# gmlewis/moonbit-flate

Hardware: AMD Instinct MI355X
Metric: GiB/s uncompressed throughput (encode), 64 KiB blocks, deflate-fast (higher is better)
Workload: dtype u8; 1 GPU; 16384 x 65536 B independent streams per GPU (1.000 GiB/GPU), S-text, deflate-fast, parity not checked in this run; streams_per_gpu=16384, stream_len=65536, kind=text, compressed_bytes_per_gpu=488295363, gather=none, parity_checked_streams=0

## Files before the change

### moonbit-flate_amd/build.py

```python
import os
import subprocess
import sys

HERE = os.path.dirname(os.path.abspath(__file__))
ROOT = os.path.dirname(HERE)
CSRC = os.path.join(HERE, "csrc")
LIB_DIR = os.path.join(HERE, "lib")
LIB_PATH = os.path.join(LIB_DIR, "libflate_hip.so")

SOURCES = ["lz77_kernels.hip",  "huff_pack_kernels.hip", "compact_kernels.hip",
           "inflate_kernels.hip", "splice_kernels.hip", "flate_api.hip", "flate_api_deflate.hip", "flate_api_inflate.hip", "gather.hip", "checksum.hip",
           "frame_kernels.hip", "chain_kernels.hip", "bgzf_kernels.hip", "bgzf_range_kernels.hip", "gzip_kernels.hip", "one_kernels.hip", "one_seek_kernels.hip", "gzfile_kernels.hip", "zip_kernels.hip", "flate_api_zip.hip", "synth.cpp"]
HEADERS = ["flate_common.h", "flate_kernels.h", "flate_ctx.h", "api_checks.h", "deflate_plan.h", "inflate_route.h", "checksum_clip.h", "bgzf_rule.h", "bgzf_range_rule.h", "gzip_rule.h", "gzfile_rule.h", "deflate_block_rule.h", "window_compose.h", "seek_index_rule.h", "zip_rule.h", "zip_kernels.h", "block_scan.h", "chain_rule.h", "chain_walk.h", "carve.h", "lz77_device.h",
           "inflate_spec_kernel.inc", "inflate_stream_kernel.inc", "one_probe_kernel.inc", os.path.join(ROOT, "include", "flate_hip.h")]


GROUPS = {
    "lz77": ["lz77_kernels.hip", "lz77_device.h", "flate_api_deflate.hip", "deflate_plan.h"],
    "huff": ["huff_pack_kernels.hip", "compact_kernels.hip", "splice_kernels.hip", "flate_api_deflate.hip", "deflate_plan.h", "block_scan.h"],
    "inflate": ["inflate_kernels.hip", "inflate_spec_kernel.inc", "inflate_stream_kernel.inc", "flate_api_inflate.hip",
                "inflate_route.h", "one_probe_kernel.inc", "one_kernels.hip", "one_seek_kernels.hip", "seek_index_rule.h", "gzfile_kernels.hip", "gzfile_rule.h",
                "deflate_block_rule.h", "window_compose.h", "chain_kernels.hip", "chain_walk.h", "chain_rule.h", "carve.h", "block_scan.h"],
    "checksum": ["checksum.hip", "checksum_clip.h", "block_scan.h", "carve.h"],
    "frame": ["frame_kernels.hip", "bgzf_kernels.hip", "bgzf_range_kernels.hip", "bgzf_rule.h", "bgzf_range_rule.h",
              "gzip_kernels.hip", "gzip_rule.h", "gzfile_kernels.hip", "gzfile_rule.h",
              "zip_kernels.hip", "zip_kernels.h", "zip_rule.h", "flate_api_zip.hip", "checksum.hip", "checksum_clip.h", "flate_api_inflate.hip",
              "inflate_route.h", "flate_api_deflate.hip", "deflate_plan.h", "block_scan.h",
              "chain_kernels.hip", "chain_walk.h", "chain_rule.h", "carve.h"],
}
SHARED = ["flate_common.h", "flate_kernels.h", "flate_ctx.h", "api_checks.h", "flate_api.hip"]


def _hash_files(names):
    import hashlib
    h = hashlib.sha256()
    for n in sorted(names):
        f = n if os.path.isabs(n) else os.path.join(CSRC, n)
        if os.path.exists(f):
            h.update(os.path.basename(f).encode() + b"\0")
            h.update(open(f, "rb").read())
    return h.hexdigest()[:12]


def source_hash(flags_by_source=None):
    import hashlib
    everything = SOURCES + [h for h in HEADERS]
    parts = ["all:" + _hash_files(everything)]
    for g, files in GROUPS.items():
        parts.append(g + ":" + _hash_files(files + SHARED))
    if flags_by_source:
        desc = ";".join("%s=%s" % (k, " ".join(v)) for k, v in sorted(flags_by_source.items()))
        parts.append("flags:" + hashlib.sha256(desc.encode()).hexdigest()[:8])
    return ";".join(parts)


def id_component(build_id, group):
    for part in (build_id or "").split(";"):
        k, _, v = part.partition(":")
        if k == group:
            return v
    return None


def _stale(lib_path=None):
    lib_path = lib_path or LIB_PATH
    if not os.path.exists(lib_path):
        return True
    t = os.path.getmtime(lib_path)
    deps = [os.path.join(CSRC, s) for s in SOURCES] + \
           [h if os.path.isabs(h) else os.path.join(CSRC, h) for h in HEADERS]
    return any(os.path.getmtime(d) > t for d in deps if os.path.exists(d))


OBJ_DIR = os.path.join(ROOT, "build", "obj")
TEST_LIB_PATH = os.path.join(LIB_DIR, "libflate_hip_testbuild.so")
TEST_BUILD_FLAGS = {"gather.hip": ["-DFLATE_HIP_TEST_BUILD"]}


def _compile_objects(hipcc, flags_by_source, verbose):
    import hashlib
    from concurrent.futures import ThreadPoolExecutor
    os.makedirs(OBJ_DIR, exist_ok=True)
    hdr_hash = _hash_files([h for h in HEADERS])
    base = ["-O3", "-std=c++17", "--offload-arch=gfx950", "-fPIC", "-I" + os.path.join(ROOT, "include"), "-I" + CSRC]
    build_id = {"flate_api.hip": ["-DFLATE_HIP_BUILD_ID=\"%s\"" % source_hash(flags_by_source)]}
    jobs = []
    for src in SOURCES:
        path = os.path.join(CSRC, src)
        if not os.path.exists(path):
            continue
        flags = base + build_id.get(src, []) + flags_by_source.get(src, [])
        key = hashlib.sha256((hdr_hash + "\0" + " ".join(flags) + "\0").encode() + open(path, "rb").read()).hexdigest()[:16]
        obj = os.path.join(OBJ_DIR, "%s-%s.o" % (os.path.splitext(src)[0], key))
        jobs.append((path, obj, flags))

    def one(job):
        path, obj, flags = job
        if not os.path.exists(obj):
            tmp = "%s.%d.tmp" % (obj, os.getpid())
            cmd = [hipcc] + flags + ["-c", path, "-o", tmp]
            if verbose:
                print(" ".join(cmd), file=sys.stderr)
            subprocess.check_call(cmd)
            os.replace(tmp, obj)
        return obj

    with ThreadPoolExecutor(max_workers=min(8, os.cpu_count() or 1)) as pool:
        return list(pool.map(one, jobs))


def _link(hipcc, objs, out, verbose):
    tmp = "%s.%d.tmp" % (out, os.getpid())
    cmd = [hipcc, "--offload-arch=gfx950", "-fPIC", "-shared"] + objs + ["-o", tmp, "-lpthread", "-ldl"]
    if verbose:
        print(" ".join(cmd), file=sys.stderr)
    subprocess.check_call(cmd)
    os.replace(tmp, out)


def build(force=False, verbose=False):
    if not force and not _stale():
        return LIB_PATH
    os.makedirs(LIB_DIR, exist_ok=True)
    hipcc = os.environ.get("HIPCC", "/opt/rocm/bin/hipcc")
    _link(hipcc, _compile_objects(hipcc, {}, verbose), LIB_PATH, verbose)
    return LIB_PATH


def build_test(force=False, verbose=False):
    if not force and not _stale(TEST_LIB_PATH):
        return TEST_LIB_PATH
    os.makedirs(LIB_DIR, exist_ok=True)
    hipcc = os.environ.get("HIPCC", "/opt/rocm/bin/hipcc")
    _link(hipcc, _compile_objects(hipcc, TEST_BUILD_FLAGS, verbose), TEST_LIB_PATH, verbose)
    return TEST_LIB_PATH


if __name__ == "__main__":
    print(build(force="--force" in sys.argv, verbose=True))
    if "--test" in sys.argv:
        print(build_test(force="--force" in sys.argv, verbose=True))
```

### moonbit-flate_amd/csrc/lz77_device.h

```cpp
#pragma once

#include "flate_kernels.h"

namespace flate {

constexpr int kDenseKeep = 61;
static_assert(kDenseKeep >= 0 && kDenseKeep <= 61, "an event must start at a lane that leaves it a scan lane (a + 2 <= 63)");
#ifndef FLATE_LZ_SWEEP_EVERY
#define FLATE_LZ_SWEEP_EVERY 20480
#endif
#ifndef FLATE_LZ_SPAN_MAX
#define FLATE_LZ_SPAN_MAX 4096
#endif
#ifndef FLATE_LZ_MARKER_BACK
#define FLATE_LZ_MARKER_BACK 36864
#endif
constexpr uint32_t kSweepEvery = FLATE_LZ_SWEEP_EVERY, kSpanMax = FLATE_LZ_SPAN_MAX, kMarkerBack = FLATE_LZ_MARKER_BACK;
static_assert(kMarkerBack > 32768u && kSweepEvery + kSpanMax + 66u + 258u + kMarkerBack < 65536u && kSpanMax >= 64u,
              "16-bit modular table slots: sweep period + batch span + marker distance must stay below 2^16");

FLATE_D uint32_t ld32(const uint8_t *p) {
  uint32_t v;
  __builtin_memcpy(&v, p, 4);
  return v;
}

FLATE_D uint32_t ld_partial(const uint8_t *p, int rem) {
  uint32_t v = p[0];
  if (rem > 1) v |= (uint32_t)p[1] << 8;
  if (rem > 2) v |= (uint32_t)p[2] << 16;
  return v;
}

FLATE_D uint32_t rdlane(uint32_t v, int lane) {
  return (uint32_t)__builtin_amdgcn_readlane((int)v, lane);
}

struct ChunkGeom {
  const uint8_t *stream;
  uint64_t len;
  uint32_t nchunks;
  uint32_t chunk0;
  uint64_t mbase;
};

FLATE_D ChunkGeom stream_geom(const LzParams &P, uint32_t sid) {
  ChunkGeom g;
  uint64_t a = P.in_off[sid], b = P.in_off[sid + 1];
  g.stream = P.in + a;
  g.len = b - a;
  g.chunk0 = P.chunk_base[sid];
  g.nchunks = P.chunk_base[sid + 1] - g.chunk0;
  g.mbase = (uint64_t)g.chunk0 * kMatchCapPerChunk;
  return g;
}

FLATE_D uint64_t lanes_below(int l) { return l >= 64 ? ~0ull : ((1ull << l) - 1ull); }
FLATE_D uint64_t lanes_upto(int l) { return l >= 63 ? ~0ull : ((1ull << (l + 1)) - 1ull); }
FLATE_D int ffs64(uint64_t m) { return m ? __builtin_ctzll(m) : 64; }

template <int CTRL, int ROW_MASK>
FLATE_D uint32_t dpp_or(uint32_t v) {
  return v | (uint32_t)__builtin_amdgcn_update_dpp(0, (int)v, CTRL, ROW_MASK, 0xf, false);
}
FLATE_D uint32_t wave_or(uint32_t v) {
  v = dpp_or<0x111, 0xf>(v);
  v = dpp_or<0x112, 0xf>(v);
  v = dpp_or<0x114, 0xf>(v);
  v = dpp_or<0x118, 0xf>(v);
  v = dpp_or<0x142, 0xa>(v);
  v = dpp_or<0x143, 0xc>(v);
  return rdlane(v, 63);
}

FLATE_D uint4 ld128(const uint8_t *p) {
  uint4 v;
  __builtin_memcpy(&v, p, 16);
  return v;
}

FLATE_D int prefix16(uint4 a, uint4 b) {
  const uint64_t lo = (uint64_t)(a.x ^ b.x) | ((uint64_t)(a.y ^ b.y) << 32);
  const uint64_t hi = (uint64_t)(a.z ^ b.z) | ((uint64_t)(a.w ^ b.w) << 32);
  if (lo) return __builtin_ctzll(lo) >> 3;
  if (hi) return 8 + (__builtin_ctzll(hi) >> 3);
  return 16;
}

constexpr uint32_t kDictEnd = (uint32_t)kMaxStoreBlockSize;
template <bool DICT>
struct HistDict {};
template <>
struct HistDict<true> {
  const uint8_t *dict;
};
template <bool DICT>
struct Hist : HistDict<DICT> {
  const uint8_t *stream;
  FLATE_D uint8_t byte(uint32_t p) const {
    if constexpr (DICT)
      if (p < kDictEnd) return this->dict[p];
    return stream[p];
  }
  FLATE_D uint32_t w32(uint32_t p) const {
    if constexpr (!DICT) return ld32(stream + p);
    if (p >= kDictEnd) return ld32(stream + p);
    if constexpr (DICT)
      if (p + 4u <= kDictEnd) return ld32(this->dict + p);
    return (uint32_t)byte(p) | ((uint32_t)byte(p + 1) << 8) | ((uint32_t)byte(p + 2) << 16) | ((uint32_t)byte(p + 3) << 24);
  }
  FLATE_D uint32_t partial(uint32_t p, int rem) const {
    if constexpr (!DICT) return ld_partial(stream + p, rem);
    if (p >= kDictEnd) return ld_partial(stream + p, rem);
    uint32_t v = byte(p);
    if (rem > 1) v |= (uint32_t)byte(p + 1) << 8;
    if (rem > 2) v |= (uint32_t)byte(p + 2) << 16;
    return v;
  }
  FLATE_D uint4 w128(uint32_t p) const {
    if constexpr (!DICT) return ld128(stream + p);
    if (p >= kDictEnd) return ld128(stream + p);
    if constexpr (DICT)
      if (p + 16u <= kDictEnd) return ld128(this->dict + p);
    return make_uint4(w32(p), w32(p + 4), w32(p + 8), w32(p + 12));
  }
};

template <bool DICT = false>
FLATE_D int extend_match(const uint8_t *src, const Hist<DICT> hist, uint32_t W, int n, int pf,
                         uint32_t cand, int have, uint32_t compat_go, int lane) {
  if (!compat_go && cand + 4 < W) return 4;
  int limit = n - pf;
  if (limit > 258) limit = 258;
  const int o = have + 4 * lane;
  uint32_t x = 0;
  if (o < limit) {
    const int r = limit - o;
    const uint8_t *pa = src + pf + o;
    if constexpr (!DICT) {
      const uint8_t *pb = hist.stream + cand + o;
      x = r >= 4 ? (ld32(pa) ^ ld32(pb)) : (ld_partial(pa, r) ^ ld_partial(pb, r));
    } else {
      const uint32_t pb = cand + (uint32_t)o;
      x = r >= 4 ? (ld32(pa) ^ hist.w32(pb)) : (ld_partial(pa, r) ^ hist.partial(pb, r));
    }
  }
  const uint64_t mm = __ballot(x != 0);
  if (!mm) return limit;
  const int k = __builtin_ctzll(mm);
  return have + 4 * k + (__builtin_ctz(rdlane(x, k)) >> 3);
}

}
```

### moonbit-flate_amd/csrc/lz77_kernels.hip

```cpp
#include <type_traits>

#include "lz77_device.h"

namespace flate {

__global__ __launch_bounds__(64) void lz77_serial_kernel(LzParams P) {
  __shared__ uint32_t table[kTableSize];
  const int lane = threadIdx.x;
  const uint32_t sid = P.stream_ids ? P.stream_ids[blockIdx.x] : blockIdx.x;
  for (int i = lane; i < kTableSize; i += 64) table[i] = 0;
  __syncthreads();
  if (lane != 0) return;

  const ChunkGeom g = stream_geom(P, sid);
  for (uint32_t c = 0; c < g.nchunks; ++c) {
    const uint32_t W = c * (uint32_t)kMaxStoreBlockSize;
    const uint64_t rem = g.len - W;
    const int n = rem < (uint64_t)kMaxStoreBlockSize ? (int)rem : kMaxStoreBlockSize;
    const uint8_t *src = g.stream + W;
    uint2 *mout = P.matches + g.mbase + (uint64_t)c * kMatchCapPerChunk;
    uint32_t nm = 0, sumlen = 0;

    const int s_limit = n - kInputMargin;
    int s = 0;
    uint32_t cv = ld32(src);
    bool done = false;
    while (!done) {
      int skip = 32;
      int next_s = s;
      uint32_t cand = 0;
      for (;;) {
        s = next_s;
        int step = skip >> 5;
        next_s = s + step;
        skip += step;
        if (next_s > s_limit) {
          done = true;
          break;
        }
        uint32_t h = hash4(cv);
        cand = table[h];
        uint32_t now = ld32(src + next_s);
        table[h] = W + (uint32_t)s + 1;
        bool ok = cand != 0 && (W + (uint32_t)s + 1 - cand) <= (uint32_t)kMaxMatchOffset &&
                  ld32(g.stream + (cand - 1)) == cv;
        if (!ok) {
          cv = now;
          continue;
        }
        break;
      }
      if (done) break;
      for (;;) {
        const int pf = s;
        s += 4;
        const uint32_t Ac = cand - 1;
        int limit = n - s;
        if (limit > kMaxMatchTail) limit = kMaxMatchTail;
        int l = 0;
        if (P.compat_go || Ac + 4 >= W) {
          const uint8_t *a = src + s, *b = g.stream + Ac + 4;
          while (l < limit && a[l] == b[l]) ++l;
        }
        mout[nm] = make_uint2((uint32_t)pf, kMatchType | ((uint32_t)(l + 1) << kLengthShift) |
                                                ((W + (uint32_t)pf) - Ac - 1));
        ++nm;
        sumlen += (uint32_t)l + 4;
        s += l;
        if (s >= s_limit) {
          done = true;
          break;
        }
        uint32_t x0 = ld32(src + s - 1), x1 = ld32(src + s);
        table[hash4(x0)] = W + (uint32_t)s;
        uint32_t h1 = hash4(x1);
        cand = table[h1];
        table[h1] = W + (uint32_t)s + 1;
        bool ok = cand != 0 && (W + (uint32_t)s + 1 - cand) <= (uint32_t)kMaxMatchOffset &&
                  ld32(g.stream + (cand - 1)) == x1;
        if (!ok) {
          cv = ld32(src + s + 1);
          s += 1;
          break;
        }
      }
    }
    P.chunk_nmatch[g.chunk0 + c] = nm;
    P.chunk_ntok[g.chunk0 + c] = (uint32_t)n - sumlen + nm;
  }
}


#ifdef FLATE_LZ_STAMPS
#define STAMP(var) const uint64_t var = __builtin_amdgcn_s_memtime()
#define STAMP_ADD(acc, t1, t0) acc += (t1) - (t0)
#else
#define STAMP(var)
#define STAMP_ADD(acc, t1, t0)
#endif


FLATE_D uint64_t same_slot_lanes(uint32_t h, uint64_t among) {
  uint32_t lo = (uint32_t)among, hi = (uint32_t)(among >> 32);
#pragma unroll
  for (int k = 0; k < kTableBits; ++k) {
    uint32_t bm = (uint32_t)((int32_t)(h << (31 - k)) >> 31);
    asm volatile("" : "+v"(bm));
    const uint64_t m = __ballot(bm != 0);
    lo &= ~((uint32_t)m ^ bm);
    hi &= ~((uint32_t)(m >> 32) ^ bm);
  }
  return ((uint64_t)hi << 32) | lo;
}

#ifndef FLATE_LZ_TAG_SLOTS
#define FLATE_LZ_TAG_SLOTS 16384
#endif
constexpr uint32_t kTagSlots = FLATE_LZ_TAG_SLOTS;
static_assert(kTagSlots % 1024 == 0 && kTagSlots <= (uint32_t)kTableSize, "whole rounds of 64 lanes x 16 slots");
FLATE_D uint32_t tag_of(uint32_t cv) { return ((cv * 0x1e35a7bdu) >> 16) & 3u; }
FLATE_D bool tag_says_no(const uint32_t *tags, uint32_t h, uint32_t cv) {
  if (kTagSlots < (uint32_t)kTableSize && h >= kTagSlots) return false;
  return ((tags[h >> 4] >> (2u * (h & 15u))) & 3u) != tag_of(cv);
}
FLATE_D void tag_set(uint32_t *tags, uint32_t h, uint32_t t) {
  if (kTagSlots < (uint32_t)kTableSize && h >= kTagSlots) return;
  const uint32_t sh = 2u * (h & 15u);
  atomicAnd(&tags[h >> 4], ~(3u << sh));
  atomicOr(&tags[h >> 4], t << sh);
}

constexpr int kLzDictStream = 1, kLzDictPrime = 2;
template <bool MULTI, bool GUEST = false, int DMODE = 0, bool HOOKS = false>
FLATE_D void lz77_stream(const LzParams &P, const uint32_t sid, uint16_t *table, const int lane,
                         const uint32_t c_begin = 0, const uint32_t c_end = 0xffffffffu,
                         uint32_t *sweep_io = nullptr, uint32_t *tags = nullptr,
                         const LzDictParams *DP = nullptr) {
  using E = uint16_t;
  constexpr bool PRIME = DMODE == kLzDictPrime, DICT = DMODE == kLzDictStream;
  static_assert(DMODE == 0 || MULTI, "a dictionary puts the payload behind position 65535: modular slots");
  uint32_t prime_w = 0, prime_n = 0;
  if constexpr (PRIME) {
    prime_n = (uint32_t)__builtin_amdgcn_readfirstlane((int)DP->dict_len[sid]);
    prime_w = kDictEnd - prime_n;
  }
  if (tags && c_begin == 0)
    for (int i = lane; i < (int)kTagSlots / 16; i += 64) tags[i] = 0;
  if (c_begin == 0) {
    uint4 *t4 = reinterpret_cast<uint4 *>(table);
    const uint32_t fill = MULTI ? (((prime_w - kMarkerBack + 1u) & 0xffffu) * 0x10001u) : 0u;
    const uint4 z = make_uint4(fill, fill, fill, fill);
    for (int i = lane; i < (int)(kTableSize * sizeof(E) / 16); i += 64) t4[i] = z;
  }
  __syncthreads();
  volatile E *vtable = table;
  constexpr uint32_t kEMask = 0xffffu;
  uint32_t next_sweep = (sweep_io && c_begin != 0) ? *sweep_io : prime_w + kSweepEvery;
  auto sweep = [&](uint32_t R) {
    uint32_t *t32 = reinterpret_cast<uint32_t *>(table);
    const uint32_t marker = (R - kMarkerBack + 1u) & 0xffffu;
    static_assert(kTableSize / 2 % (64 * 16) == 0, "table = whole rounds of 16 dwords per lane");
    for (int i0 = lane; i0 < kTableSize / 2; i0 += 64 * 16) {
      uint32_t w[16];
#pragma unroll
      for (int k = 0; k < 16; ++k) w[k] = t32[i0 + 64 * k];
#pragma unroll
      for (int k = 0; k < 16; ++k) {
        const uint32_t v = w[k];
        const uint32_t d0 = (R + 1u - v) & 0xffffu, d1 = (R + 1u - (v >> 16)) & 0xffffu;
        const uint32_t lo = (d0 == 0 || d0 > 32768u) ? marker : (v & 0xffffu);
        const uint32_t hi = (d1 == 0 || d1 > 32768u) ? marker : (v >> 16);
        t32[i0 + 64 * k] = lo | (hi << 16);
      }
    }
    __syncthreads();
    next_sweep = R + kSweepEvery;
  };

  ChunkGeom g;
  Hist<DICT> hist;
  if constexpr (PRIME) {
    g.stream = DP->dict_buf + DP->dict_at[sid] - prime_w;
    g.len = kDictEnd;
    g.nchunks = 1;
    g.chunk0 = 0;
    g.mbase = 0;
  } else {
    g = stream_geom(P, sid);
  }
  if constexpr (DICT) {
    const uint32_t slot = DP->slot_of[sid];
    hist.dict = DP->dict_buf + DP->dict_at[slot] - (kDictEnd - DP->dict_len[slot]);
    g.stream -= kDictEnd;
    g.len += kDictEnd;
  }
  hist.stream = g.stream;
  const uint16_t *scan_tab = P.scan_off;
  uint32_t pf_sink = 0;
#ifdef FLATE_LZ_FINISH
  const uint64_t fin_t0 = __builtin_amdgcn_s_memrealtime();
#endif

  const uint32_t w0 = (uint32_t)__builtin_amdgcn_readfirstlane((int)P.win0);
  const uint32_t c_stop = c_end < w0 + g.nchunks ? c_end : w0 + g.nchunks;
  for (uint32_t c = c_begin; c < c_stop; ++c) {
    const uint32_t W = PRIME ? prime_w : c * (uint32_t)kMaxStoreBlockSize;
    const uint64_t rem_len = g.len - W;
    const int n = rem_len < (uint64_t)kMaxStoreBlockSize ? (int)rem_len : kMaxStoreBlockSize;
    const uint8_t *src = g.stream + W;
    uint2 *mout = P.matches + g.mbase + (uint64_t)(c - w0) * kMatchCapPerChunk;
    uint32_t nm = 0;
    uint32_t acc_len = 0;
    const int s_limit = n - kInputMargin;

    int s = -1;
    bool sparse = false;
    int scan_base = 0, e_idx = 0;
    bool done = false;
    uint4 own_pre = make_uint4(0, 0, 0, 0);
    bool pre_valid = false;
    int pf_blk = -2;
#ifdef FLATE_LZ_STAMPS
    uint64_t st_load = 0, st_dup = 0, st_ev = 0, st_commit = 0, st_sparse = 0, st_nb = 0, st_ext = 0;
#endif

    const uint64_t spec_full =
        (2ull << lane) | (lane + 2 < 64 ? ((0x00000000ffffffffull << (lane + 2)) | (0x5555555500000000ull << (lane + 2)))
                                        : 0ull);
    auto no_progress = [&]() {
      if (lane == 0) atomicExch(P.status, kStatusNoProgress);
      done = true;
    };
    uint32_t h_nb = 0, h_acc = 0;
    int h_e = 0;
    bool moved = true;
    while (!done) {
      if (!moved) {
        no_progress();
        break;
      }
      if constexpr (HOOKS) h_acc = acc_len, h_e = e_idx;
      if (!sparse) {
        auto dense_batch = [&](auto interior_tag) {
          constexpr bool INTERIOR = decltype(interior_tag)::value;
        STAMP(t0);
        const int B = s - 1;
        if (MULTI) {
          const uint32_t first = W + (uint32_t)(B < 0 ? 0 : B);
          if (first >= next_sweep) sweep(first);
        }
        const int q = B + lane;
        const bool e1 = INTERIOR || (q >= 0 && q + 1 <= s_limit);
        const bool e2 = INTERIOR || (q >= 0 && q + 2 <= s_limit);
        const uint64_t E1 = INTERIOR ? ~0ull : __ballot(e1), E2 = INTERIOR ? ~0ull : __ballot(e2);
        const uint32_t A1 = W + (uint32_t)q + 1;
        uint4 own = make_uint4(0, 0, 0, 0);
        uint32_t h = 0, old = 0;
        bool maybe = false;
        if (e1) {
          own = pre_valid ? own_pre : ld128(src + q);
          h = hash4(own.x);
          maybe = !tags || !tag_says_no(tags, h, own.x);
          if (maybe) old = table[h];
        }
        pre_valid = false;
        const uint32_t dist = MULTI ? ((A1 - old) & 0xffffu) : (A1 - old);
        const bool inr = maybe && (MULTI ? dist != 0 : old != 0) && dist <= (uint32_t)kMaxMatchOffset;
        const uint32_t cand_abs = A1 - 1u - dist;
        uint4 cb = own;
        if (inr) cb = hist.w128(cand_abs);
        if ((B >> 8) != pf_blk) {
          pf_blk = B >> 8;
          int pq = (B & ~255) + 1024 + 4 * lane;
          if (pq > n - 4) pq = n - 4;
          pf_sink = ld32(src + pq);
        }
        uint64_t DUPall = 0, DUP = 0;
        uint64_t eq = 0;
        if (GUEST) {
          eq = same_slot_lanes(h, E1);
          if (!e1) eq = 0;
          DUPall = __ballot((eq & ~(1ull << lane)) != 0);
          DUP = __ballot((eq & lanes_below(lane)) != 0);
        }
        asm volatile("" ::: "memory");
        if (!GUEST && e1) table[h] = (E)A1;
        asm volatile("" ::: "memory");
        const uint32_t rb = (!GUEST && e1) ? (uint32_t)table[h] : (A1 & kEMask);
        asm volatile("" ::: "memory");
        const bool loser = rb != (A1 & kEMask);
        const uint64_t LM = GUEST ? 0ull : __ballot(loser);
        if (!GUEST) DUPall = LM;
        if (LM) {
          const int wl = (int)((rb - (W + (uint32_t)B + 1u)) & kEMask);
          uint64_t m = LM;
          while (m) {
            const int x = __builtin_ctzll(m);
            const int w = (int)rdlane((uint32_t)wl, x);
            const uint64_t Lw = __ballot(loser && wl == w);
            DUPall |= 1ull << w;
            if (__popcll(Lw) == 1)
              DUP |= 1ull << (w > x ? w : x);
            else
              DUP |= Lw | (1ull << w);
            m &= ~Lw;
          }
        }
        STAMP(t1);
        const int bsh = lane + 2;
        uint64_t specR;
        if (E1 == ~0ull && E2 == ~0ull) {
          specR = spec_full;
        } else {
          specR = (E1 & (2ull << lane)) | (bsh < 64 ? (((0x00000000ffffffffull << bsh) & E1) |
                                                       ((0x5555555500000000ull << bsh) & E2))
                                                    : 0ull);
        }
        const uint64_t dupR = DUP & specR;
        const int fd = dupR ? __builtin_ctzll(dupR) : 64;
        const int mlen = inr ? prefix16(own, cb) : 0;
        const uint64_t OK = __ballot(mlen >= 4);
        const bool cross = MULTI && !P.compat_go && cand_abs + 4 < W;
        const int tot_self = cross ? 4 : mlen;
        uint32_t rec_tok = kMatchType | ((uint32_t)(tot_self - 3) << kLengthShift) | (dist - 1u);
        uint32_t ev;
        {
          const uint64_t okR = OK & specR & ~DUP;
          const int fv = okR ? __builtin_ctzll(okR) : 64;
          const int tf = __shfl(tot_self, fv & 63);
          const bool slow = !(fv < fd) || tf >= 16;
          const bool ends = B + fv + tf >= s_limit;
          const int nxt = fv + tf - 1;
#ifdef FLATE_LZ_TERM_SHORTCUT
          const bool off_batch = INTERIOR && fv == 64 && fd == 64;
#else
          constexpr bool off_batch = false;
#endif
          ev = (uint32_t)(fv & 127) | ((uint32_t)tf << 8) | (slow ? 1u << 16 : 0u) |
               (ends ? 1u << 17 : 0u) | ((ends || nxt > kDenseKeep) ? 1u << 18 : 0u) | (off_batch ? 1u << 19 : 0u) |
               ((uint32_t)(nxt & 255) << 24);
        }
        STAMP(t2);

        auto fast_inserts = [&](uint64_t vis) -> uint64_t {
          const uint64_t below_me = vis & lanes_upto(lane);
          const int j = below_me ? 63 - __builtin_clzll(below_me) : 0;
          const int fvj = (int)(__shfl(ev, j) & 127u);
          const int d = lane - j, o = d - 2;
          const bool sched = (d <= 1 || o < 32) ? e1 : (((o & 1) == 0) ? e2 : false);
          return __ballot(below_me != 0 && sched && lane <= fvj);
        };
        uint64_t INS = 0, M = 0, MF = 0;
        uint64_t VISall = 0;
        int a = 0;
        for (;;) {
          uint32_t x, tmp;
          uint64_t VIS = 0, MFl = 0;
          int a_s = __builtin_amdgcn_readfirstlane(a);
          STAMP(tc0);
          asm volatile(
              "1:\n\t"
              "s_nop 1\n\t"
              "v_readlane_b32 %[x], %[ev], %[a]\n\t"
              "s_nop 3\n\t"
              "s_bitcmp1_b32 %[x], 16\n\t"
              "s_cbranch_scc1 2f\n\t"
              "s_bitset1_b64 %[vis], %[a]\n\t"
              "s_and_b32 %[t], %[x], 0x7f\n\t"
              "s_bitset1_b64 %[mf], %[t]\n\t"
              "s_lshr_b32 %[a], %[x], 24\n\t"
              "s_bitcmp1_b32 %[x], 18\n\t"
              "s_cbranch_scc1 2f\n\t"
              "s_nop 1\n\t"
              "v_readlane_b32 %[x], %[ev], %[a]\n\t"
              "s_nop 3\n\t"
              "s_bitcmp1_b32 %[x], 16\n\t"
              "s_cbranch_scc1 2f\n\t"
              "s_bitset1_b64 %[vis], %[a]\n\t"
              "s_and_b32 %[t], %[x], 0x7f\n\t"
              "s_bitset1_b64 %[mf], %[t]\n\t"
              "s_lshr_b32 %[a], %[x], 24\n\t"
              "s_bitcmp1_b32 %[x], 18\n\t"
              "s_cbranch_scc0 1b\n\t"
              "2:\n\t"
              : [x] "=&s"(x), [a] "+s"(a_s), [vis] "+s"(VIS), [mf] "+s"(MFl), [t] "=&s"(tmp)
              : [ev] "v"(ev)
              : "scc");
          a = a_s;
          MF |= MFl;
          STAMP(tc1);
          STAMP_ADD(st_sparse, tc1, tc0);
          VISall |= VIS;
          s = B + a + 1;
          if (!(x & (1u << 16))) {
            if (x & (1u << 17)) done = true;
            break;
          }
#ifdef FLATE_LZ_TERM_SHORTCUT
          if (INTERIOR && (x & (1u << 19)) && a != 0) break;
#endif
          STAMP(tg0);
          const uint64_t FINS = fast_inserts(VISall);
          const uint64_t a_ins = E1 & (1ull << a);
          const int b = a + 2;
          const uint64_t full = 0x55555555ffffffffull << b;
          const uint64_t scanR = ((0x00000000ffffffffull << b) & E1) | ((0x5555555500000000ull << b) & E2);
          const uint64_t R = (E1 & (2ull << a)) | scanR;
          const bool scan_ended = scanR != full;

          uint64_t T = 0, rem = R;
          int f = 64, have = 0;
          uint32_t cand = 0;
          for (;;) {
            const int fv = ffs64(OK & rem & ~DUP), fd = ffs64(DUP & rem);
            if (fv < fd) {
              f = fv;
              cand = rdlane(cand_abs, fv);
              have = (int)rdlane((uint32_t)mlen, fv);
              T |= rem & lanes_upto(fv);
              break;
            }
            if (fd == 64) {
              T |= rem;
              break;
            }
            T |= rem & lanes_below(fd);
            const uint32_t hfd = rdlane(h, fd);
            const uint64_t G = __ballot(e1 && h == hfd) & (INS | FINS | T | a_ins) & lanes_below(fd);
            bool v;
            uint32_t cnd;
            int ml;
            if (G) {
              const int i = 63 - __builtin_clzll(G);
              v = rdlane(own.x, i) == rdlane(own.x, fd);
              cnd = W + (uint32_t)(B + i);
              const uint4 oi = make_uint4(rdlane(own.x, i), rdlane(own.y, i), rdlane(own.z, i),
                                          rdlane(own.w, i));
              const uint4 of = make_uint4(rdlane(own.x, fd), rdlane(own.y, fd), rdlane(own.z, fd),
                                          rdlane(own.w, fd));
              ml = prefix16(of, oi);
            } else {
              v = (OK >> fd) & 1;
              cnd = rdlane(cand_abs, fd);
              ml = (int)rdlane((uint32_t)mlen, fd);
            }
            T |= 1ull << fd;
            if (v) {
              f = fd;
              cand = cnd;
              have = ml;
              break;
            }
            rem &= ~lanes_upto(fd);
          }

          if (f == 64) {
            if (scan_ended) {
              INS |= T | a_ins;
              done = true;
            } else if (a == 0) {
              INS |= T | a_ins;
              sparse = true;
              scan_base = s + 1;
              e_idx = 47;
            }
            break;
          }
          INS |= T | a_ins;
          const int pf = B + f;
          int total;
          if (have < 16)
            total = (!P.compat_go && cand + 4 < W) ? 4 : have;
          else
            total = extend_match(src, hist, W, n, pf, cand, 16, P.compat_go, lane);
          M |= 1ull << f;
          if (lane == f) {
            rec_tok = kMatchType | ((uint32_t)(total - 3) << kLengthShift) | ((W + (uint32_t)pf) - cand - 1);
            acc_len += (uint32_t)total;
          }
          s = pf + total;
          STAMP(tg1);
          STAMP_ADD(st_ext, tg1, tg0);
          if (s >= s_limit) {
            done = true;
            break;
          }
          a = s - 1 - B;
          if (a > kDenseKeep) break;
        }
        M |= MF;
        INS |= fast_inserts(VISall);
        if constexpr (HOOKS) {
          if (P.inject_stall != 0 && ++h_nb == P.inject_stall) {
            s = B + 1, e_idx = h_e, sparse = false, done = false;
            acc_len = h_acc;
            M = MF = INS = 0;
          }
        }
        STAMP(t3);
        if (!done && !sparse) {
          const int qn = s - 1 + lane;
          if (qn + 1 <= s_limit) own_pre = ld128(src + qn);
          pre_valid = true;
        }
        if ((MF >> lane) & 1) acc_len += (uint32_t)tot_self;
        if (!PRIME && ((M >> lane) & 1))
          {
            const unsigned long long rec = (unsigned long long)(uint32_t)q | ((unsigned long long)rec_tok << 32);
            __builtin_nontemporal_store(
                rec, reinterpret_cast<unsigned long long *>(mout + nm + (uint32_t)__popcll(M & lanes_below(lane))));
          }
        nm += (uint32_t)__popcll(M);
        asm volatile("" ::: "memory");
        if (GUEST) {
          if (e1 && ((INS >> lane) & 1) && (eq & INS & ~lanes_upto(lane)) == 0) {
            table[h] = (E)A1;
            if (tags) tag_set(tags, h, tag_of(own.x));
          }
        } else {
          if (e1 && (((DUPall | ~INS) >> lane) & 1)) table[h] = (E)old;
          uint64_t dm = DUPall & INS;
          while (dm) {
            const int k = __builtin_ctzll(dm);
            asm volatile("" ::: "memory");
            if (lane == k) table[h] = (E)A1;
            dm &= dm - 1;
          }
        }
        asm volatile("" ::: "memory");
        STAMP(t4);
        STAMP_ADD(st_dup, t1, t0);
        STAMP_ADD(st_load, t2, t1);
        STAMP_ADD(st_ev, t3, t2);
        STAMP_ADD(st_commit, t4, t3);
#ifdef FLATE_LZ_STAMPS
        st_nb += 1;
#endif
        };
        const int s0 = s;
        if (s - 1 >= 0 && s - 1 + 65 <= s_limit)
          dense_batch(std::true_type{});
        else
          dense_batch(std::false_type{});
        moved = (s != s0) | sparse | done;
      } else {
        const int e = e_idx + lane;
        int p, step;
        if (e < kScanClosedForm) {
          p = scan_base + scan_off_small(e, &step);
        } else {
          const int ec = e < P.scan_len - 1 ? e : P.scan_len - 2;
          const int o0 = scan_tab[ec], o1 = scan_tab[ec + 1];
          p = scan_base + o0 + (e - ec) * 65536;
          step = o1 - o0;
        }
        const bool exists_all = p + step <= s_limit;
        const int p0 = (int)rdlane((uint32_t)p, 0);
        const bool exists = exists_all && (!MULTI || (uint32_t)(p - p0) < kSpanMax);
        const int nall = __popcll(__ballot(exists_all));
        const int nexist = __popcll(__ballot(exists));
        if (nall == 0) break;
        if (MULTI && W + (uint32_t)p0 >= next_sweep) sweep(W + (uint32_t)p0);

        uint32_t cv = 0, h = 0, old = 0;
        if (exists) {
          cv = ld32(src + p);
          h = hash4(cv);
          old = vtable[h];
        }
        const uint32_t A1 = W + (uint32_t)p + 1;
        const uint32_t dist = MULTI ? ((A1 - old) & 0xffffu) : (A1 - old);
        const uint32_t cand_abs = A1 - 1u - dist;
        bool ok = false;
        if (exists && (MULTI ? dist != 0 : old != 0) && dist <= (uint32_t)kMaxMatchOffset)
          ok = hist.w32(cand_abs) == cv;
        const uint64_t V = __ballot(ok);
        const int f0 = ffs64(V);

        const int lim = f0 < nexist - 1 ? f0 : nexist - 1;
        const bool ins = lane <= lim;
        uint64_t C;
        if (GUEST) {
          const uint64_t eqs = same_slot_lanes(h, __ballot(ins));
          C = __ballot(ins && (eqs & ~(1ull << lane)) != 0);
          if (C == 0 && ins) {
            vtable[h] = (E)A1;
            if (tags) tag_set(tags, h, tag_of(cv));
          }
        } else {
          if (ins) vtable[h] = (E)A1;
          const uint32_t rb = ins ? (uint32_t)vtable[h] : (A1 & kEMask);
          C = __ballot(rb != (A1 & kEMask));
        }

        int f = f0;
        uint32_t cand = 0;
        if (C == 0) {
          if (f0 < 64) cand = rdlane(cand_abs, f0);
        } else {
          if (!GUEST && ins) vtable[h] = (E)old;
          f = 64;
          for (int e2 = 0; e2 < nexist; ++e2) {
            const uint32_t he = rdlane(h, e2);
            const uint32_t pe1 = rdlane(A1, e2);
            const uint32_t cur =
                (uint32_t)__builtin_amdgcn_readfirstlane((int)(uint32_t)vtable[he]);
            vtable[he] = (E)pe1;
            if (tags && lane == e2) tag_set(tags, h, tag_of(cv));
            bool v;
            uint32_t cnd;
            if (cur == rdlane(old, e2)) {
              v = (V >> e2) & 1;
              cnd = rdlane(cand_abs, e2);
            } else {
              const uint64_t m = __ballot(exists && (A1 & kEMask) == cur);
              v = false;
              cnd = 0;
              if (m) {
                const int i = __builtin_ctzll(m);
                v = rdlane(cv, i) == rdlane(cv, e2);
                cnd = rdlane(A1, i) - 1u;
              }
            }
            if (v) {
              f = e2;
              cand = cnd;
              break;
            }
          }
        }
        if (f == 64) {
          if (nexist == nall && nall < 64) break;
          if (nexist == 0) {
            no_progress();
            break;
          }
          e_idx += nexist;
          continue;
        }
        const int pf = (int)rdlane((uint32_t)p, f);
        const int total = extend_match(src, hist, W, n, pf, cand, 4, P.compat_go, lane);
        if (!PRIME && lane == 0)
          mout[nm] = make_uint2((uint32_t)pf, kMatchType | ((uint32_t)(total - 3) << kLengthShift) |
                                                  ((W + (uint32_t)pf) - cand - 1));
        ++nm;
        if (lane == 0) acc_len += (uint32_t)total;
        s = pf + total;
        sparse = false;
        if (s >= s_limit) done = true;
      }
    }
    uint32_t sumlen = acc_len;
    for (int d = 32; d >= 1; d >>= 1) sumlen += __shfl_xor(sumlen, d);
    if (pf_sink == 0x9e3779b9u && P.debug) P.debug[0] = pf_sink;
    if (!PRIME && lane == 0) {
      P.chunk_nmatch[g.chunk0 + c - w0] = nm;
      P.chunk_ntok[g.chunk0 + c - w0] = (uint32_t)n - sumlen + nm;
#ifdef FLATE_LZ_STAMPS
      if (P.debug) {
        uint64_t *d = P.debug + (uint64_t)(g.chunk0 + c - w0) * 8;
        d[0] = st_dup; d[1] = st_load; d[2] = st_ev; d[3] = st_commit; d[4] = st_nb; d[5] = nm;
        d[6] = st_ext; d[7] = st_sparse;
      }
#endif
    }
  }
  if (sweep_io) *sweep_io = next_sweep;
#ifdef FLATE_LZ_FINISH
  if (lane == 0 && P.debug && c_begin == 0) {
    uint64_t *d = P.debug + (uint64_t)g.chunk0 * 8;
    d[0] = fin_t0;
    d[1] = __builtin_amdgcn_s_memrealtime();
    d[2] = ((uint64_t)(GUEST ? 1u : 0u) << 32) | blockIdx.x;
  }
#endif
}

FLATE_D void all_lanes_here(const LzParams &P, int lane) {
  const uint64_t here = __ballot(true);
  if (here != ~0ull && lane == (int)__builtin_ctzll(here)) atomicExch(P.status, kStatusLanesLost);
}

struct UqUnit {
  uint32_t q;
  uint32_t c;
  bool ok;
};

template <bool HOOKS>
FLATE_D UqUnit uq_pop(const LzParams &P, const uint32_t push_word, int lane) {
  uint32_t t = 0;
  if (lane == 0) {
    if (push_word != 0 && !(push_word & 0x80000000u)) {
      const uint32_t k = __hip_atomic_fetch_add(P.uq_ctr + 1, 1u, __ATOMIC_RELAXED, __HIP_MEMORY_SCOPE_AGENT);
      bool dropped = false;
      if constexpr (HOOKS) dropped = k + 1u - P.queue_end == P.inject_drop_push;
      if (!dropped)
        __hip_atomic_store(P.uq_ready + k, push_word, __ATOMIC_RELAXED, __HIP_MEMORY_SCOPE_AGENT);
    }
    t = __hip_atomic_fetch_add(P.uq_ctr, 1u, __ATOMIC_RELAXED, __HIP_MEMORY_SCOPE_AGENT);
  }
  t = (uint32_t)__builtin_amdgcn_readfirstlane((int)t);
  const uint32_t units = P.uq_units;
  uint32_t v = 0;
  if (t < units) {
    for (uint32_t polls = 0;; ++polls) {
      uint32_t x = 0;
      if (lane == 0) x = __hip_atomic_load(P.uq_ready + t, __ATOMIC_RELAXED, __HIP_MEMORY_SCOPE_AGENT);
      v = (uint32_t)__builtin_amdgcn_readfirstlane((int)x);
      if (v != 0) break;
      if (polls >= P.spin_limit) break;
      __builtin_amdgcn_s_sleep(16);
    }
    if (v == 0 && lane == 0) atomicExch(P.status, kStatusUqTimeout);
    if (lane == 0) (void)__hip_atomic_load(P.uq_ready + t, __ATOMIC_ACQUIRE, __HIP_MEMORY_SCOPE_AGENT);
    asm volatile("s_waitcnt vmcnt(0)" ::: "memory");
  }
  __syncthreads();
  UqUnit u;
  v = (uint32_t)__builtin_amdgcn_readfirstlane((int)v);
  u.ok = v != 0;
  u.q = (v >> 15) - 1u;
  u.c = v & 0x7fffu;
  return u;
}

__global__ void uq_init_kernel(uint32_t *ready, uint32_t *ctr, uint32_t n_streams, uint32_t n_units) {
  const uint32_t i = blockIdx.x * blockDim.x + threadIdx.x;
  if (i < n_units) ready[i] = i < n_streams ? ((i + 1u) << 15) : 0u;
  if (i == 0) {
    ctr[0] = 0;
    ctr[1] = n_streams;
  }
}

template <bool GUEST, bool HOOKS>
FLATE_D uint32_t uq_run(const LzParams &P, const UqUnit u, uint16_t *table, int lane, uint32_t *tags = nullptr) {
  const uint32_t sid = (uint32_t)__builtin_amdgcn_readfirstlane((int)P.stream_ids[u.q]);
  const uint32_t nch = (uint32_t)__builtin_amdgcn_readfirstlane((int)(P.chunk_base[sid + 1] - P.chunk_base[sid]));
  uint32_t *home = reinterpret_cast<uint32_t *>(P.uq_tables + (size_t)u.q * kTableSize);
  uint32_t *work = reinterpret_cast<uint32_t *>(table);
  uint32_t clock = 0;
  if (u.c != 0) {
    clock = (uint32_t)__builtin_amdgcn_readfirstlane(
        (int)__hip_atomic_load(P.uq_sweep + u.q, __ATOMIC_RELAXED, __HIP_MEMORY_SCOPE_AGENT));
    const uint8_t *stream = P.in + P.in_off[sid];
    const uint32_t W = u.c * (uint32_t)kMaxStoreBlockSize;
    if (tags) {
      for (int i = lane; i < (int)kTagSlots / 16; i += 64) tags[i] = 0;
      __syncthreads();
    }
    static_assert(kTableSize / 2 % (64 * 16) == 0, "table = whole rounds of 16 dwords per lane");
    for (int i0 = lane; i0 < kTableSize / 2; i0 += 64 * 16) {
      uint32_t w[16];
#pragma unroll
      for (int k = 0; k < 16; ++k) w[k] = __hip_atomic_load(home + i0 + 64 * k, __ATOMIC_RELAXED, __HIP_MEMORY_SCOPE_AGENT);
#pragma unroll
      for (int k = 0; k < 16; ++k) work[i0 + 64 * k] = w[k];
      if (tags) {
#pragma unroll
        for (int half = 0; half < 2; ++half) {
          uint32_t cv[16];
#pragma unroll
          for (int j = 0; j < 16; ++j) {
            const uint32_t slot = (w[half * 8 + j / 2] >> (16 * (j & 1))) & 0xffffu;
            const uint32_t back = (W + 1u - slot) & 0xffffu;
            cv[j] = (back != 0u && back <= W) ? ld32(stream + (W - back)) : 0xffffffffu;
          }
#pragma unroll
          for (int j = 0; j < 16; ++j) {
            const uint32_t slot = (w[half * 8 + j / 2] >> (16 * (j & 1))) & 0xffffu;
            const uint32_t back = (W + 1u - slot) & 0xffffu;
            const uint32_t h = 2u * (uint32_t)(i0 + 64 * (half * 8 + j / 2)) + (uint32_t)(j & 1);
            if (back != 0u && back <= W && h < kTagSlots) atomicOr(&tags[h >> 4], tag_of(cv[j]) << (2u * (h & 15u)));
          }
        }
      }
    }
  }
  asm volatile("s_waitcnt vmcnt(0) lgkmcnt(0)" ::: "memory");
  __syncthreads();
  lz77_stream<true, GUEST, 0, HOOKS>(P, sid, table, lane, u.c, u.c + 1, &clock, tags);
  asm volatile("s_waitcnt vmcnt(0) lgkmcnt(0)" ::: "memory");
  __syncthreads();
  if (u.c + 1 < nch) {
    for (int i0 = lane; i0 < kTableSize / 2; i0 += 64 * 16) {
      uint32_t w[16];
#pragma unroll
      for (int k = 0; k < 16; ++k) w[k] = work[i0 + 64 * k];
#pragma unroll
      for (int k = 0; k < 16; ++k) __hip_atomic_store(home + i0 + 64 * k, w[k], __ATOMIC_RELAXED, __HIP_MEMORY_SCOPE_AGENT);
    }
    if (lane == 0) __hip_atomic_store(P.uq_sweep + u.q, clock, __ATOMIC_RELAXED, __HIP_MEMORY_SCOPE_AGENT);
    asm volatile("s_waitcnt vmcnt(0) lgkmcnt(0)" ::: "memory");
    __syncthreads();
    return ((u.q + 1u) << 15) | (u.c + 1u);
  }
  return 0x80000000u | u.q;
}

FLATE_D void table_copy(uint16_t *dst, const uint16_t *src, int lane) {
  const uint32_t *s = reinterpret_cast<const uint32_t *>(src);
  uint32_t *d = reinterpret_cast<uint32_t *>(dst);
  static_assert(kTableSize / 2 % (64 * 16) == 0, "table = whole rounds of 16 dwords per lane");
  for (int i0 = lane; i0 < kTableSize / 2; i0 += 64 * 16) {
    uint32_t w[16];
#pragma unroll
    for (int k = 0; k < 16; ++k) w[k] = s[i0 + 64 * k];
#pragma unroll
    for (int k = 0; k < 16; ++k) d[i0 + 64 * k] = w[k];
  }
}

FLATE_D void dict_snapshot_load(const LzDictParams &DP, uint32_t sid, uint16_t *table, uint32_t *clock, int lane) {
  const uint32_t slot = (uint32_t)__builtin_amdgcn_readfirstlane((int)DP.slot_of[sid]);
  table_copy(table, DP.tables + (size_t)slot * kTableSize, lane);
  *clock = (uint32_t)__builtin_amdgcn_readfirstlane((int)DP.clocks[slot]);
  asm volatile("s_waitcnt vmcnt(0) lgkmcnt(0)" ::: "memory");
  __syncthreads();
}


template <bool MULTI, bool GUEST, bool DICT, bool COUNT, bool HOOKS>
FLATE_D void stream_loop(const LzParams P, uint16_t *table, uint32_t *tags, const LzDictParams *DP, int lane) {
  uint32_t mine = 0;
  for (bool first = true;; first = false) {
    uint32_t q;
    if (GUEST || P.queue) {
      q = 0;
      if (lane == 0) q = atomicAdd(P.queue, 1u);
      q = (uint32_t)__builtin_amdgcn_readfirstlane((int)q);
      if (q >= P.queue_end) break;
    } else {
      if (!first) break;
      q = blockIdx.x;
    }
    __syncthreads();
    if constexpr (DICT) {
      const uint32_t sid = (uint32_t)__builtin_amdgcn_readfirstlane((int)P.stream_ids[q]);
      uint32_t clock = 0;
      dict_snapshot_load(*DP, sid, table, &clock, lane);
      lz77_stream<true, GUEST, kLzDictStream, HOOKS>(P, sid, table, lane, 1, 0xffffffffu, &clock, nullptr, DP);
    } else {
      lz77_stream<MULTI, GUEST, 0, HOOKS>(P, (GUEST || P.stream_ids) ? P.stream_ids[q] : q, table, lane, 0, 0xffffffffu,
                                          nullptr, tags);
    }
    __syncthreads();
    all_lanes_here(P, lane);
    if (COUNT) ++mine;
  }
  if (COUNT && P.taken && lane == 0) __hip_atomic_fetch_add(P.taken, mine, __ATOMIC_RELAXED, __HIP_MEMORY_SCOPE_AGENT);
}

template <bool GUEST, bool COUNT, bool HOOKS>
FLATE_D void unit_loop(const LzParams P, uint16_t *table, uint32_t *tags, int lane) {
  uint32_t push_word = 0;
  uint32_t mine = 0;
  for (;;) {
    const UqUnit u = uq_pop<HOOKS>(P, push_word, lane);
    if (__builtin_amdgcn_readfirstlane((int)u.ok) == 0) break;
    push_word = (uint32_t)__builtin_amdgcn_readfirstlane((int)uq_run<GUEST, HOOKS>(P, u, table, lane, tags));
    all_lanes_here(P, lane);
    if (COUNT) ++mine;
  }
  if (COUNT && P.taken && lane == 0) __hip_atomic_fetch_add(P.taken, mine, __ATOMIC_RELAXED, __HIP_MEMORY_SCOPE_AGENT);
}

template <bool MULTI, bool HOOKS>
__global__ __launch_bounds__(64) void lz77_wave_kernel(LzParams P) {
  __shared__ uint16_t table[kTableSize];
  if (MULTI && P.uq_ready)
    unit_loop<false, true, HOOKS>(P, table, nullptr, threadIdx.x);
  else
    stream_loop<MULTI, false, false, true, HOOKS>(P, table, nullptr, nullptr, threadIdx.x);
}

FLATE_D uint16_t *guest_table(const LzParams &P) {
  return reinterpret_cast<uint16_t *>(P.gtables) + (size_t)blockIdx.x * kTableSize;
}

template <bool MULTI, bool HOOKS>
__global__ __launch_bounds__(64) void lz77_guest_kernel(LzParams P) {
  if (blockIdx.x >= P.gtable_blocks) return;
  __shared__ uint32_t tags[kTagSlots / 16];
  uint16_t *table = guest_table(P);
  const int lane = threadIdx.x;
  if (MULTI && P.uq_ready) {
    unit_loop<true, false, HOOKS>(P, table, tags, lane);
    return;
  }
  stream_loop<MULTI, true, false, false, HOOKS>(P, table, tags, nullptr, lane);
}

template <bool HOOKS>
__global__ __launch_bounds__(64) void lz77_wave_dict_kernel(LzParams P, LzDictParams DP) {
  __shared__ uint16_t table[kTableSize];
  stream_loop<true, false, true, false, HOOKS>(P, table, nullptr, &DP, threadIdx.x);
}

template <bool HOOKS>
__global__ __launch_bounds__(64) void lz77_guest_dict_kernel(LzParams P, LzDictParams DP) {
  if (blockIdx.x >= P.gtable_blocks) return;
  stream_loop<true, true, true, false, HOOKS>(P, guest_table(P), nullptr, &DP, threadIdx.x);
}

__global__ __launch_bounds__(64) void lz77_dict_prime_kernel(LzParams P, LzDictParams DP) {
  __shared__ uint16_t table[kTableSize];
  const int lane = threadIdx.x;
  const uint32_t slot = blockIdx.x;
  uint32_t clock = 0;
  lz77_stream<true, false, kLzDictPrime>(P, slot, table, lane, 0, 1, &clock, nullptr, &DP);
  __syncthreads();
  table_copy(DP.tables + (size_t)slot * kTableSize, table, lane);
  if (lane == 0) DP.clocks[slot] = clock;
}


__global__ __launch_bounds__(64) void lz77_resume_kernel(LzParams P, uint16_t *table_io, uint32_t *clock_io,
                                                          uint32_t nwin, uint32_t rebase, uint32_t forget) {
  __shared__ uint16_t table[kTableSize];
  const int lane = threadIdx.x;
  uint32_t clock = 0;
  if (P.win0 != 0 && forget) {
    const uint32_t W = P.win0 * (uint32_t)kMaxStoreBlockSize;
    const uint32_t fill = ((W - kMarkerBack + 1u) & 0xffffu) * 0x10001u;
    uint4 *dst = reinterpret_cast<uint4 *>(table);
    for (int i = lane; i < (int)(kTableSize * sizeof(uint16_t) / 16); i += 64) dst[i] = make_uint4(fill, fill, fill, fill);
    clock = W + kSweepEvery;
  } else if (P.win0 != 0) {
    table_copy(table, table_io, lane);
    clock = *clock_io - rebase;
    if (rebase) {
      __syncthreads();
      uint32_t *t32 = reinterpret_cast<uint32_t *>(table);
      const uint32_t d16 = rebase & 0xffffu;
      for (int i = lane; i < kTableSize / 2; i += 64) {
        const uint32_t v = t32[i];
        t32[i] = ((v - d16) & 0xffffu) | ((((v >> 16) - d16) & 0xffffu) << 16);
      }
    }
  }
  __syncthreads();
  lz77_stream<true>(P, 0, table, lane, P.win0, P.win0 + nwin, &clock);
  __syncthreads();
  table_copy(table_io, table, lane);
  if (lane == 0) *clock_io = clock;
}

template __global__ void lz77_wave_kernel<false, false>(LzParams);
template __global__ void lz77_wave_kernel<true, false>(LzParams);
template __global__ void lz77_guest_kernel<false, false>(LzParams);
template __global__ void lz77_guest_kernel<true, false>(LzParams);
template __global__ void lz77_wave_dict_kernel<false>(LzParams, LzDictParams);
template __global__ void lz77_guest_dict_kernel<false>(LzParams, LzDictParams);
template __global__ void lz77_wave_kernel<false, true>(LzParams);
template __global__ void lz77_wave_kernel<true, true>(LzParams);
template __global__ void lz77_guest_kernel<false, true>(LzParams);
template __global__ void lz77_guest_kernel<true, true>(LzParams);
template __global__ void lz77_wave_dict_kernel<true>(LzParams, LzDictParams);
template __global__ void lz77_guest_dict_kernel<true>(LzParams, LzDictParams);

}
```

Before: 58.10 GiB/s.

## Precompute two-hop event pairs so the scalar LZ77 chase jumps two events per readlane

Each lane now builds a second packed word that combines its own match event with the event it points to, fetched with one cross-lane shuffle. The serial scalar chase loop reads this pair word, so each dependent v_readlane plus its nop padding advances two events instead of one. This shortens the latency-bound pointer chain through the wavefront. In exchange it adds a shuffle and some bit packing per batch, and the asm hard-codes the new bit layout. A host-side reference model of the chase is added, and the unused FLATE_LZ_TERM_SHORTCUT path is removed.

```diff
diff --git a/moonbit-flate_amd/build.py b/moonbit-flate_amd/build.py
--- a/moonbit-flate_amd/build.py
+++ b/moonbit-flate_amd/build.py
@@ -11,12 +11,12 @@
 SOURCES = ["lz77_kernels.hip",  "huff_pack_kernels.hip", "compact_kernels.hip",
            "inflate_kernels.hip", "splice_kernels.hip", "flate_api.hip", "flate_api_deflate.hip", "flate_api_inflate.hip", "gather.hip", "checksum.hip",
            "frame_kernels.hip", "chain_kernels.hip", "bgzf_kernels.hip", "bgzf_range_kernels.hip", "gzip_kernels.hip", "one_kernels.hip", "one_seek_kernels.hip", "gzfile_kernels.hip", "zip_kernels.hip", "flate_api_zip.hip", "synth.cpp"]
-HEADERS = ["flate_common.h", "flate_kernels.h", "flate_ctx.h", "api_checks.h", "deflate_plan.h", "inflate_route.h", "checksum_clip.h", "bgzf_rule.h", "bgzf_range_rule.h", "gzip_rule.h", "gzfile_rule.h", "deflate_block_rule.h", "window_compose.h", "seek_index_rule.h", "zip_rule.h", "zip_kernels.h", "block_scan.h", "chain_rule.h", "chain_walk.h", "carve.h", "lz77_device.h",
+HEADERS = ["flate_common.h", "flate_kernels.h", "flate_ctx.h", "api_checks.h", "deflate_plan.h", "inflate_route.h", "checksum_clip.h", "bgzf_rule.h", "bgzf_range_rule.h", "gzip_rule.h", "gzfile_rule.h", "deflate_block_rule.h", "window_compose.h", "seek_index_rule.h", "zip_rule.h", "zip_kernels.h", "block_scan.h", "chain_rule.h", "chain_walk.h", "carve.h", "lz77_device.h", "lz77_chase_rule.h",
            "inflate_spec_kernel.inc", "inflate_stream_kernel.inc", "one_probe_kernel.inc", os.path.join(ROOT, "include", "flate_hip.h")]
 
 
 GROUPS = {
-    "lz77": ["lz77_kernels.hip", "lz77_device.h", "flate_api_deflate.hip", "deflate_plan.h"],
+    "lz77": ["lz77_kernels.hip", "lz77_device.h", "lz77_chase_rule.h", "flate_api_deflate.hip", "deflate_plan.h"],
     "huff": ["huff_pack_kernels.hip", "compact_kernels.hip", "splice_kernels.hip", "flate_api_deflate.hip", "deflate_plan.h", "block_scan.h"],
     "inflate": ["inflate_kernels.hip", "inflate_spec_kernel.inc", "inflate_stream_kernel.inc", "flate_api_inflate.hip",
                 "inflate_route.h", "one_probe_kernel.inc", "one_kernels.hip", "one_seek_kernels.hip", "seek_index_rule.h", "gzfile_kernels.hip", "gzfile_rule.h",
diff --git a/moonbit-flate_amd/csrc/lz77_chase_rule.h b/moonbit-flate_amd/csrc/lz77_chase_rule.h
--- /dev/null
+++ b/moonbit-flate_amd/csrc/lz77_chase_rule.h
@@ -0,0 +1,84 @@
+#pragma once
+
+#include <stdint.h>
+
+#if defined(__HIPCC__)
+#define CHASE_HD __host__ __device__ inline
+#else
+#define CHASE_HD inline
+#endif
+
+namespace flate {
+
+constexpr int kDenseKeep = 61;
+static_assert(kDenseKeep >= 0 && kDenseKeep <= 61, "an event must start at a lane that leaves it a scan lane (a + 2 <= 63)");
+
+constexpr uint32_t kEvSlow = 1u << 16, kEvEnds = 1u << 17, kEvStop = 1u << 18;
+constexpr int kEvNextShift = 24;
+
+constexpr uint32_t kPairNone = 1u << 15;
+constexpr int kPairFv1Shift = 8, kPairA1Shift = 19, kPairNextShift = 25;
+static_assert(kDenseKeep < 64 && 63 + 15 - 1 < 128, "a1 takes six bits and the next start lane seven");
+
+CHASE_HD uint32_t chase_pair(uint32_t lane, uint32_t ev_mine, uint32_t ev_next) {
+  const bool stop = (ev_mine & kEvStop) != 0, next_slow = (ev_next & kEvSlow) != 0;
+  const bool two = !stop && !next_slow;
+  const uint32_t last = two ? ev_next : ev_mine;
+#ifndef CHASE_MUTANT_IGNORE_STOP2
+  uint32_t bits = last & (kEvEnds | kEvStop);
+#else
+  uint32_t bits = last & (two ? kEvEnds : (kEvEnds | kEvStop));
+#endif
+  if (!stop && next_slow) bits = kEvSlow | kEvStop;
+  const uint32_t w = (last & 63u) | ((ev_mine & 63u) << kPairFv1Shift) | bits |
+                     ((two ? ev_mine >> kEvNextShift : lane) << kPairA1Shift) |
+                     ((last >> kEvNextShift) << kPairNextShift);
+  return (ev_mine & kEvSlow) ? (kPairNone | kEvSlow) : w;
+}
+
+struct ChaseEnd {
+  uint64_t vis, mf;
+  uint32_t a, exit;
+};
+CHASE_HD uint32_t chase_exit_bits(uint32_t x) { return (x & kEvSlow) ? kEvSlow : (x & kEvEnds); }
+
+CHASE_HD ChaseEnd chase_single(const uint32_t *ev, uint32_t a) {
+  ChaseEnd r = {0, 0, a, 0};
+  for (;;) {
+    const uint32_t x = ev[r.a];
+    r.exit = chase_exit_bits(x);
+    if (x & kEvSlow) return r;
+    r.vis |= 1ull << r.a;
+    r.mf |= 1ull << (x & 63u);
+    r.a = x >> kEvNextShift;
+    if (x & kEvStop) return r;
+  }
+}
+
+CHASE_HD ChaseEnd chase_paired(const uint32_t *ev, const uint32_t *ev2, uint32_t a) {
+  ChaseEnd r = {0, 0, a, 0};
+  for (;;) {
+    const uint32_t x = ev2[r.a];
+    if (x & kPairNone) {
+      const uint32_t y = ev[r.a];
+      r.exit = chase_exit_bits(y);
+      if (y & kEvSlow) return r;
+      r.vis |= 1ull << r.a;
+      r.mf |= 1ull << (y & 63u);
+      r.a = y >> kEvNextShift;
+      if (y & kEvStop) return r;
+      continue;
+    }
+    r.exit = chase_exit_bits(x);
+#ifndef CHASE_MUTANT_DROP_MIDDLE
+    r.vis |= (1ull << r.a) | (1ull << ((x >> kPairA1Shift) & 63u));
+#else
+    r.vis |= 1ull << r.a;
+#endif
+    r.mf |= (1ull << ((x >> kPairFv1Shift) & 63u)) | (1ull << (x & 63u));
+    r.a = x >> kPairNextShift;
+    if (x & kEvStop) return r;
+  }
+}
+
+}
diff --git a/moonbit-flate_amd/csrc/lz77_device.h b/moonbit-flate_amd/csrc/lz77_device.h
--- a/moonbit-flate_amd/csrc/lz77_device.h
+++ b/moonbit-flate_amd/csrc/lz77_device.h
@@ -1,11 +1,10 @@
 #pragma once
 
 #include "flate_kernels.h"
+#include "lz77_chase_rule.h"
 
 namespace flate {
 
-constexpr int kDenseKeep = 61;
-static_assert(kDenseKeep >= 0 && kDenseKeep <= 61, "an event must start at a lane that leaves it a scan lane (a + 2 <= 63)");
 #ifndef FLATE_LZ_SWEEP_EVERY
 #define FLATE_LZ_SWEEP_EVERY 20480
 #endif
diff --git a/moonbit-flate_amd/csrc/lz77_kernels.hip b/moonbit-flate_amd/csrc/lz77_kernels.hip
--- a/moonbit-flate_amd/csrc/lz77_kernels.hip
+++ b/moonbit-flate_amd/csrc/lz77_kernels.hip
@@ -331,15 +331,11 @@
           const bool slow = !(fv < fd) || tf >= 16;
           const bool ends = B + fv + tf >= s_limit;
           const int nxt = fv + tf - 1;
-#ifdef FLATE_LZ_TERM_SHORTCUT
-          const bool off_batch = INTERIOR && fv == 64 && fd == 64;
-#else
-          constexpr bool off_batch = false;
-#endif
           ev = (uint32_t)(fv & 127) | ((uint32_t)tf << 8) | (slow ? 1u << 16 : 0u) |
-               (ends ? 1u << 17 : 0u) | ((ends || nxt > kDenseKeep) ? 1u << 18 : 0u) | (off_batch ? 1u << 19 : 0u) |
+               (ends ? 1u << 17 : 0u) | ((ends || nxt > kDenseKeep) ? 1u << 18 : 0u) |
                ((uint32_t)(nxt & 255) << 24);
         }
+        const uint32_t ev2 = chase_pair((uint32_t)lane, ev, (uint32_t)__shfl((int)ev, (int)((ev >> kEvNextShift) & 63u)));
         STAMP(t2);
 
         auto fast_inserts = [&](uint64_t vis) -> uint64_t {
@@ -358,34 +354,33 @@
           uint64_t VIS = 0, MFl = 0;
           int a_s = __builtin_amdgcn_readfirstlane(a);
           STAMP(tc0);
+#define FLATE_LZ_CHASE_STEP(BRANCH)                                                           \
+              "s_nop 1\n\t"                                                                   \
+              "v_readlane_b32 %[x], %[ev2], %[a]\n\t"                                         \
+              "s_nop 3\n\t"                                                                   \
+              "s_bitcmp1_b32 %[x], 15\n\t"                                                    \
+              "s_cbranch_scc1 2f\n\t"                                                         \
+              "s_bitset1_b64 %[vis], %[a]\n\t"                                                \
+              "s_bfe_u32 %[t], %[x], 0x60013\n\t"               \
+              "s_bitset1_b64 %[vis], %[t]\n\t"                                                \
+              "s_bfe_u32 %[t], %[x], 0x60008\n\t"               \
+              "s_bitset1_b64 %[mf], %[t]\n\t"                                                 \
+              "s_and_b32 %[t], %[x], 0x7f\n\t"                                                \
+              "s_bitset1_b64 %[mf], %[t]\n\t"                                                 \
+              "s_lshr_b32 %[a], %[x], 25\n\t"                                                 \
+              "s_bitcmp1_b32 %[x], 18\n\t" BRANCH
+          static_assert(kPairNone == 1u << 15 && kPairFv1Shift == 8 && kPairA1Shift == 19 && kPairNextShift == 25 &&
+                            kEvSlow == 1u << 16 && kEvEnds == 1u << 17 && kEvStop == 1u << 18,
+                        "the loop below names the pair word's bits");
           asm volatile(
               "1:\n\t"
-              "s_nop 1\n\t"
-              "v_readlane_b32 %[x], %[ev], %[a]\n\t"
-              "s_nop 3\n\t"
-              "s_bitcmp1_b32 %[x], 16\n\t"
-              "s_cbranch_scc1 2f\n\t"
-              "s_bitset1_b64 %[vis], %[a]\n\t"
-              "s_and_b32 %[t], %[x], 0x7f\n\t"
-              "s_bitset1_b64 %[mf], %[t]\n\t"
-              "s_lshr_b32 %[a], %[x], 24\n\t"
-              "s_bitcmp1_b32 %[x], 18\n\t"
-              "s_cbranch_scc1 2f\n\t"
-              "s_nop 1\n\t"
-              "v_readlane_b32 %[x], %[ev], %[a]\n\t"
-              "s_nop 3\n\t"
-              "s_bitcmp1_b32 %[x], 16\n\t"
-              "s_cbranch_scc1 2f\n\t"
-              "s_bitset1_b64 %[vis], %[a]\n\t"
-              "s_and_b32 %[t], %[x], 0x7f\n\t"
-              "s_bitset1_b64 %[mf], %[t]\n\t"
-              "s_lshr_b32 %[a], %[x], 24\n\t"
-              "s_bitcmp1_b32 %[x], 18\n\t"
-              "s_cbranch_scc0 1b\n\t"
+              FLATE_LZ_CHASE_STEP("s_cbranch_scc1 2f\n\t")
+              FLATE_LZ_CHASE_STEP("s_cbranch_scc0 1b\n\t")
               "2:\n\t"
               : [x] "=&s"(x), [a] "+s"(a_s), [vis] "+s"(VIS), [mf] "+s"(MFl), [t] "=&s"(tmp)
-              : [ev] "v"(ev)
+              : [ev2] "v"(ev2)
               : "scc");
+#undef FLATE_LZ_CHASE_STEP
           a = a_s;
           MF |= MFl;
           STAMP(tc1);
@@ -396,9 +391,6 @@
             if (x & (1u << 17)) done = true;
             break;
           }
-#ifdef FLATE_LZ_TERM_SHORTCUT
-          if (INTERIOR && (x & (1u << 19)) && a != 0) break;
-#endif
           STAMP(tg0);
           const uint64_t FINS = fast_inserts(VISall);
           const uint64_t a_ins = E1 & (1ull << a);
```

Result: faster. 58.78 GiB/s (median of 6 runs) (+1.2%).
